# sikang/motion_primitive_library

Hardware: AMD Instinct MI355X
Metric: node-expansions/s (frontier x |U| pair evaluations per second) (higher is better)
Workload: dtype f64; 1 GPU; C4: 3D VoxelMapUtil 512^3, Control::ACC |U|=729 (9^3), 64k-node synthetic frontier; frontier=random, frontier_nodes=65536, frontier_nodes_per_gpu=65536, controls=729, dim=3, map_cells=134217728, device=AMD Radeon Graphics (gfx950:sramecc+:xnack-), compute_units=256, kernel=expand_lex_kernel

## Files before the change

motion_primitive_library_amd/build.py:

```python
import os
import shutil
import subprocess
import sys

HERE = os.path.dirname(os.path.abspath(__file__))
CSRC = os.path.join(HERE, "csrc")
LIB = os.path.join(CSRC, "libmplx.so")
SOURCES = ["expand_kernel.hip", "expand_tile_kernel.hip", "expand_grid_kernel.hip", "expand_lex_kernel.hip", "expand_pair_kernel.hip", "map_prep_kernel.hip", "map_prep_api.cpp", "map_util_kernel.hip", "map_util_api.cpp", "rollout_kernel.hip", "rollout_api.cpp", "ray_kernel.hip", "ray_api.cpp", "traj_kernel.hip", "traj_api.cpp", "solve_kernel.hip", "solve_api.cpp", "limits_kernel.hip", "limits_api.cpp", "scale_kernel.hip", "scale_api.cpp", "conflict_kernel.hip", "conflict_api.cpp", "reserve_kernel.hip", "reserve_api.cpp", "reserve_poly_kernel.hip", "reserve_poly_api.cpp", "wait_kernel.hip", "wait_api.cpp", "table_kernel.hip", "table_api.cpp", "open_kernel.hip", "open_best_kernel.hip", "open_rekey_kernel.hip", "open_api.cpp", "field_kernel.hip", "field_api.cpp", "heur_kernel.hip", "heur_api.cpp", "replan_kernel.hip", "replan_api.cpp", "post_kernel.hip", "identity_kernel.hip", "post_api.cpp", "edge_kernel.hip", "edge_api.cpp", "mplx_api.cpp", "lists_route.cpp", "yaw_pin.cpp", "lists_host.cpp", "planner_capi.cpp", "pack_kernel.hip", "store_model_kernel.hip", "lists_copy_api.cpp", "pack_api.cpp", "comm_api.cpp"]
HEADERS = ["mplx_internal.h", "mplx_ctx.h", "mplx_stage.h", "mplx_device_common.h", "mplx_pair_device.h", "mplx_grid_common.h", "mplx_poly.h", "mplx_traj_device.h", "mplx_limits_math.h", "mplx_scale_math.h", "mplx_heur_math.h", "mplx_open_heur.h", "host_planner.hpp", "host_lpastar.hpp", os.path.join("..", "..", "include", "mplx.h"), os.path.join("..", "..", "include", "mplx_debug.h"), os.path.join("..", "..", "include", "mplx_map_util.h"), os.path.join("..", "..", "include", "mplx_rollout.h"), os.path.join("..", "..", "include", "mplx_ray.h"), os.path.join("..", "..", "include", "mplx_traj.h"), os.path.join("..", "..", "include", "mplx_table.h"), os.path.join("..", "..", "include", "mplx_open.h"), os.path.join("..", "..", "include", "mplx_multi.h"), os.path.join("..", "..", "include", "mplx_replan.h"), os.path.join("..", "..", "include", "mplx_replan_timed.h"), os.path.join("..", "..", "include", "mplx_prior.h"), os.path.join("..", "..", "include", "mplx_solve.h"), os.path.join("..", "..", "include", "mplx_limits.h"), os.path.join("..", "..", "include", "mplx_scale.h"), os.path.join("..", "..", "include", "mplx_conflict.h"), os.path.join("..", "..", "include", "mplx_reserve.h"), os.path.join("..", "..", "include", "mplx_reserve_poly.h"), os.path.join("..", "..", "include", "mplx_wait.h"), os.path.join("..", "..", "include", "mplx_field.h"), os.path.join("..", "..", "include", "mplx_heur.h"), os.path.join("..", "..", "include", "mplx_best.h"), os.path.join("..", "..", "include", "mplx_anytime.h")]
ARCH = "gfx950"


def hipcc_path():
    for cand in (os.environ.get("HIPCC"), shutil.which("hipcc"), "/opt/rocm/bin/hipcc"):
        if cand and os.path.exists(cand):
            return cand
    raise RuntimeError("hipcc not found (set HIPCC or install ROCm under /opt/rocm)")


def _obj_dir():
    d = os.path.join(CSRC, "build")
    os.makedirs(d, exist_ok=True)
    return d


def is_stale():
    if not os.path.exists(LIB):
        return True
    t = os.path.getmtime(LIB)
    deps = [os.path.join(CSRC, s) for s in SOURCES + HEADERS]
    return any(os.path.getmtime(d) > t for d in deps)

# ... 61 lines not shown
```

motion_primitive_library_amd/csrc/expand_lex_kernel.hip:

```cpp
#include "mplx_internal.h"
#include "mplx_device_common.h"

namespace mplx {

using namespace dev;

constexpr int kLexWPB = 4;
constexpr int kLexBT = 64 * kLexWPB;
constexpr int kLexTabStride = 64;
constexpr int kLexUB8 = 8;

constexpr int kShUval = 0;
__host__ __device__ constexpr int lex_sh_tc(int TS) { return TS == 32 ? 768 : 384; }
__host__ __device__ constexpr int lex_sh_tt(int TS) { return lex_sh_tc(TS) + 64; }
__host__ __device__ constexpr int lex_ts(int ndp) { return ndp <= 8 ? 8 : (ndp <= 16 ? 16 : 32); }

__host__ __device__ constexpr int lex_fixed_bytes(int D, int K, int TS) {
  const int F = 4 * D + 2, KQ = K == 3 ? 4 : K;
  int w = (F * 8 + 15) & ~15;
  w += 128 + D * TS * 4 + D * TS * 4 * KQ + D * TS * 8 * (K - 1) + (K == 3 ? D * TS * 8 : 0) + D * TS + D * TS;
  w = (w + 15) & ~15;
  return (w + 128 + 7) & ~7;
}
__host__ __device__ constexpr int lex_tt_entries(int n_max) { return (n_max + 1) * (n_max + 2) / 2; }
// ... 511 lines not shown
        for (int i = 0; i < D; i++) {
          lo[i] = wave_reduce_minmax<false>(lo_l[i]);
          const int hi = wave_reduce_minmax<true>(hi_l[i]);
          if (hi < lo[i]) have_box = false;
          nb[i] = hi - lo[i] + 1;
        }
      }
      lex_sync();
      const int WX = (nb[0] + 31) >> 5;
      const int n_rows = nb[1] * nb[2];
      const bool fits = have_box && n_rows * WX <= A.boxcap;
      const int rot = (WX == 1) ? (lo[0] & 31) : 0;
      if (D == 2 && eager) {
        if (fits && pass == 0 && lane < nb[1]) {
          unsigned int val = e_in ? (__builtin_amdgcn_alignbit(e_a1, e_a0, e_shf) | ~e_mask) : 0xffffffffu;
          val = __builtin_amdgcn_alignbit(val, val, (32 - rot) & 31);
          s_box[lane] = val;
        }
      } else if (fits) {
        const float inv_ny = __builtin_amdgcn_rcpf((float)nb[1]);
        const int ax0 = base_c[0] + lo[0] - half;
        constexpr int SU = 4;
        const int ayb = base_c[1] + lo[1] - half, azb = (D == 3) ? base_c[2] + lo[2] - half : 0;
        for (int w = 0; w < WX; w++) {
          const int xw = ax0 + 32 * w;
          const int vlo = xw < 0 ? -xw : 0;
          const int vhi = (dims[0] - xw) < 32 ? (dims[0] - xw) : 32;
          const unsigned int mask = (vhi >= 32 ? 0xffffffffu : ((1u << (vhi > 0 ? vhi : 0)) - 1u)) & ~((1u << vlo) - 1u);
          for (int r0 = lane; r0 < n_rows; r0 += 64 * SU) {
            unsigned int a0[SU], a1[SU], shf[SU];
            bool in[SU];
#pragma unroll
            for (int u = 0; u < SU; u++) {
              const int r = r0 + 64 * u;
              const int rz = (D == 3) ? (int)(((float)r + 0.5f) * inv_ny) : 0;
              const int ry = r - rz * nb[1];
              const int ay = ayb + ry, az = azb + rz;
              in[u] = r < n_rows && vhi > vlo && ay >= 0 && ay < dims[1] && (D == 2 || (az >= 0 && az < dims[2]));
              const int64_t off = in[u] ? ((int64_t)az * dims[1] + ay) * (int64_t)dims[0] + xw : 0;
              const int64_t wi = off >> 5;
              shf[u] = (unsigned)(off & 31);
              const int64_t w0 = wi < 0 ? 0 : wi;
              const int64_t w1 = wi + 1 >= A.blk_words ? A.blk_words - 1 : wi + 1;
              a0[u] = (A.dbg & 8) ? 0u : A.blk[w0];
              a1[u] = (A.dbg & 8) ? 0u : A.blk[w1 < 0 ? 0 : w1];
            }
// ... 305 lines not shown
```

motion_primitive_library_amd/csrc/lists_route.cpp:

```cpp
#include "mplx_ctx.h"

#include <cmath>
#include <cstdio>
#include <cstdlib>

namespace mplx_detail {


template <class Args>
static void set_env(const mplx_ctx *c, Args *a) {
  a->region = c->has_region ? (const uint32_t *)c->region_bits.p : nullptr;
  a->dim0 = c->mdim[0]; a->dim1 = c->mdim[1]; a->dim2 = c->mdim[2];
  a->org0 = c->origin[0]; a->org1 = c->origin[1]; a->org2 = c->origin[2];
  a->res = c->res;
  a->dt = c->prm.dt; a->w = c->prm.w;
  a->v_max = c->prm.v_max; a->a_max = c->prm.a_max; a->j_max = c->prm.j_max;
}

template <class Args>
static void set_tables(const mplx_ctx *c, Args *a) {
  a->ttab = (const double *)c->tables.p;
  a->tcnt = (const unsigned char *)c->tables.p + kTcntOffset;
  a->Rres = c->recips[0]; a->R001 = c->recips[1]; a->R01 = c->recips[2];
}
// ... 306 lines not shown
  a->live_n = live_n;
  return MPLX_OK;
}

static int rebuild_sat(mplx_ctx *c) {
  c->sat_stale = false;
  const int d2p = c->dim == 3 ? c->mdim[2] + 1 : 2;
  const int64_t sat_n = (int64_t)(c->mdim[0] + 1) * (c->mdim[1] + 1) * d2p;
  if (c->tune.no_sat || sat_n * 4 > (16LL << 30)) return MPLX_OK;
  if (int rc = ensure(c, c->sat, (size_t)sat_n * 4)) return rc;
  HIP_TRY(c, mplx::launch_build_sat(c->dim, (const uint32_t *)c->blk.p, c->mdim, (uint32_t *)c->sat.p, c->stream));
  c->sat_ok = true;
  return MPLX_OK;
}

int ensure_blocked_bits(mplx_ctx *c) {
  if (c->blk_ok) return MPLX_OK;
  c->sat_stale = false;
  const int64_t words = (c->n_cells + 31) >> 5;
  if (int rc = ensure(c, c->blk, (size_t)words * 4)) return rc;
  HIP_TRY(c, mplx::launch_build_blocked_bits((const int8_t *)(c->has_pot ? c->pot.p : c->map.p),
                                             c->has_region ? (const uint32_t *)c->region_bits.p : nullptr, c->n_cells,
                                             c->has_pot ? 1 : 0, (uint32_t *)c->blk.p, c->stream));
  c->sat_ok = false;
  if (int rc = rebuild_sat(c)) return rc;
  c->blk_ok = true;
  return MPLX_OK;
}

int ensure_tables(mplx_ctx *c) {
  if (c->tables_ok && c->tab_dt == c->prm.dt && c->tab_res == c->res) return MPLX_OK;
  const size_t bytes = kTcntOffset + 64 + 64;
  if (int rc = ensure(c, c->tables, bytes)) return rc;
  double *ttab = (double *)c->tables.p;
  unsigned char *tcnt = (unsigned char *)c->tables.p + kTcntOffset;
  double *rec = (double *)((unsigned char *)c->tables.p + kTcntOffset + 64);
  HIP_TRY(c, hipMemsetAsync(c->tables.p, 0, bytes, c->stream));
  HIP_TRY(c, mplx::launch_make_tables(c->prm.dt, c->res, ttab, tcnt, rec, c->stream));
  HIP_TRY(c, hipMemcpyAsync(c->recips, rec, 3 * sizeof(double), hipMemcpyDeviceToHost, c->stream));
  HIP_TRY(c, hipStreamSynchronize(c->stream));
  c->tab_dt = c->prm.dt;
  c->tab_res = c->res;
  c->tables_ok = true;
  return MPLX_OK;
}

static uint32_t const_zero_rows(int dim, int control) {
  const int order = control_order(control);
  uint32_t m = 0;
  for (int b = order + 1; b <= 3; b++)
    for (int i = 0; i < dim; i++) m |= 1u << (b * dim + i);
  if (!(control & 0x10)) m |= 1u << (4 * dim);
  return m;
}

static mplx::GridArgs grid_args(mplx_ctx *c, const GridPlan &gp, const double *d_nodes, int64_t n_nodes, int64_t node_stride,
                                const mplx_succ_lists *o, uint32_t skip) {
  mplx::GridArgs a{};
  set_env(c, &a);
  set_tables(c, &a);
  set_lists(c, o, &a);
  a.blk = (const uint32_t *)c->blk.p;
  a.blk_words = (c->n_cells + 31) >> 5;
  a.pot = c->has_pot ? (const int8_t *)c->pot.p : nullptr;
  a.pot_w = c->prm.potential_weight;
  a.grad_w = c->has_pot ? c->prm.gradient_weight : 0.0;
  const bool yaw = (c->prm.control & 0x10) != 0;
  a.sat = (c->sat_ok && gp.order <= 3 && !(yaw && c->prm.wyaw > 0) && !c->tune.no_sat && gp.use_sat)
              ? (const uint32_t *)c->sat.p : nullptr;
  a.gather = gp.gather ? 1 : 0;
  a.yaw_max = c->prm.yaw_max; a.wyaw = c->prm.wyaw; a.ndy = yaw ? c->u_nd[3] : 0;
  a.uvals = (const double *)c->uvals.p + (c->u_wide ? 4 * 16 : 0);
  a.uval_stride = c->u_wide ? 32 : 16;
  a.uidx = (const uint32_t *)c->uidx.p;
  a.nd0 = c->u_nd[0]; a.nd1 = c->u_nd[1]; a.nd2 = c->u_nd[2];
  a.ndp = gp.ndp;
  a.ulex = gp.ulex;
  a.nU = c->nU;
  a.nodes = d_nodes; a.n_nodes = n_nodes; a.node_stride = node_stride;
  a.n_max = gp.n_max; a.rmax = gp.rmax; a.boxcap = gp.boxcap; a.grid_limit = gp.grid;
  a.lex = gp.lex ? 1 : 0;
  a.dbg = c->tune.dbg;
  a.l_pad = line_pad(c, a.l_nstride);
  a.l_zrows = skip;
  a.post = post_of(c, o);
  return a;
// ... 178 lines not shown
```

motion_primitive_library_amd/csrc/map_prep_api.cpp:

```cpp
#include "mplx_ctx.h"

#include <array>
#include <cmath>
#include <cstring>
#include <unordered_map>
#include <vector>

using namespace mplx_detail;

namespace {

inline int float_to_int(double pt, double origin, double res) { return (int)std::round((pt - origin) / res - 0.5); }

}

extern "C" {

int mplx_edit_map(mplx_ctx *c, const int64_t *cell_index, const int8_t *values, int64_t n) {
  if (!c) return MPLX_ERR_ARG;
  if (n < 0 || (n > 0 && (!cell_index || !values))) return fail(c, MPLX_ERR_ARG, "mplx_edit_map: bad arguments");
  if (!c->has_map) return fail(c, MPLX_ERR_STATE, "mplx_edit_map: set the map first");
  for (int64_t i = 0; i < n; i++)
    if (cell_index[i] < 0 || cell_index[i] >= c->n_cells)
      return fail(c, MPLX_ERR_ARG, "mplx_edit_map: cell index %lld outside the map of %lld cells", (long long)cell_index[i], (long long)c->n_cells);
// ... 8 lines not shown
        std::unordered_map<int64_t, int64_t> last;
        last.reserve((size_t)n * 2);
        for (int64_t i = 0; i < n; i++) last[cell_index[i]] = i;
        if ((int64_t)last.size() < n) {
          u_idx.reserve(last.size());
          u_val.reserve(last.size());
          for (int64_t i = 0; i < n; i++)
            if (last[cell_index[i]] == i) { u_idx.push_back(cell_index[i]); u_val.push_back(values[i]); }
          cell_index = u_idx.data();
          values = u_val.data();
          n = (int64_t)u_idx.size();
        }
      } catch (...) { return fail(c, MPLX_ERR_NOMEM, "mplx_edit_map: out of host memory"); }
    }
  }
  if (int rc = bind_device(c)) return rc;
  if (int rc = resolve_pending(c)) return rc;
  if (int rc = svc_stop(c)) return rc;
  StageRows s;
  const auto i_idx = s.in(cell_index, (size_t)n * 8), i_val = s.in(values, (size_t)n);
  if (int rc = stage_commit(c, &s)) return rc;
  c->map_upload_bytes += (uint64_t)n * 9;
  uint32_t *blk = (c->blk_ok && !c->has_pot) ? (uint32_t *)c->blk.p : nullptr;
  HIP_TRY(c, mplx::launch_edit_map(s.dev<int64_t>(i_idx), s.dev<int8_t>(i_val), n, c->n_cells, (int8_t *)c->map.p, blk,
                                   c->has_region ? (const uint32_t *)c->region_bits.p : nullptr, c->stream));
  if (int rc = stage_fetch(c, &s)) return rc;
  c->blk_epoch++;
  if (blk && c->sat_ok) {
    c->sat_ok = false;
    c->sat_stale = true;
  }
  return MPLX_OK;
}

int mplx_read_cells(mplx_ctx *c, int which, const int64_t *cell_index, int64_t n, int8_t *out) {
  if (!c) return MPLX_ERR_ARG;
  if (n < 0 || (n > 0 && (!cell_index || !out)) || (which != 0 && which != 1)) return fail(c, MPLX_ERR_ARG, "mplx_read_cells: bad arguments");
  if (which == 0 ? !c->has_map : !c->has_pot) return fail(c, MPLX_ERR_STATE, which == 0 ? "mplx_read_cells: no map set" : "mplx_read_cells: no potential map set");
  for (int64_t i = 0; i < n; i++)
    if (cell_index[i] < 0 || cell_index[i] >= c->n_cells)
      return fail(c, MPLX_ERR_ARG, "mplx_read_cells: cell index %lld outside the map of %lld cells", (long long)cell_index[i], (long long)c->n_cells);
  if (n == 0) return MPLX_OK;
  if (int rc = bind_device(c)) return rc;
  StageRows s;
  const auto i_idx = s.in(cell_index, (size_t)n * 8), o_val = s.out(out, (size_t)n);
  if (int rc = stage_commit(c, &s)) return rc;
  HIP_TRY(c, mplx::launch_gather_cells((const int8_t *)(which == 0 ? c->map.p : c->pot.p), s.dev<int64_t>(i_idx), n, s.dev<int8_t>(o_val), c->stream));
// ... 153 lines not shown
```

motion_primitive_library_amd/csrc/map_prep_kernel.hip:

```cpp
#include "mplx_internal.h"

namespace mplx {
namespace {

constexpr unsigned short kFar = 0xffff;

__global__ void pot_x_kernel(const int8_t *map, int d0, int d1, int d2, int c1x, int c2x, int c1y, int c2y, int c1z,
                             int c2z, int rn, unsigned short *dx2) {
  const int64_t n = (int64_t)d0 * d1 * d2;
  const int64_t g = (int64_t)blockIdx.x * blockDim.x + threadIdx.x;
  if (g >= n) return;
  const int x = (int)(g % d0);
  const int64_t row = g / d0;
  const int y = (int)(row % d1), z = (int)(row / d1);
  unsigned int best = kFar;
  if (y >= c1y && y < c2y && z >= c1z && z < c2z) {
    const int lo = max(x - rn, c1x), hi = min(x + rn, c2x - 1);
    const int8_t *r = map + row * d0;
    for (int s = lo; s <= hi; s++)
      if (r[s] > 0) {
        const unsigned int d = (unsigned)((s - x) * (s - x));
        best = d < best ? d : best;
      }
  }
// ... 52 lines not shown
  if (g >= per * n_cells_path) return;
  const int p = (int)(g / per);
  int64_t o = g - (int64_t)p * per;
  const int ox = (int)(o % bx) - rn0;
  o /= bx;
  const int oy = (int)(o % by) - rn1;
  const int oz = (int)(o / by) - rn2;
  const int x = cells[p * 3 + 0] + ox, y = cells[p * 3 + 1] + oy, z = (dim == 3) ? cells[p * 3 + 2] + oz : 0;
  if (x < 0 || x >= d0 || y < 0 || y >= d1 || z < 0 || z >= d2) return;
  const int64_t idx = x + (int64_t)d0 * y + (int64_t)d0 * d1 * z;
  atomicOr(&bits[idx >> 5], 1u << (idx & 31));
}

__global__ void unpack_region_kernel(const uint32_t *bits, int64_t n_cells, uint8_t *bytes) {
  const int64_t g = (int64_t)blockIdx.x * blockDim.x + threadIdx.x;
  if (g >= n_cells) return;
  bytes[g] = (uint8_t)((bits[g >> 5] >> (g & 31)) & 1u);
}

inline unsigned blocks_for(int64_t n) { return (unsigned)((n + 255) / 256); }


__global__ void edit_map_kernel(const int64_t *idx, const int8_t *val, int64_t n, int64_t n_cells, int8_t *map, uint32_t *blk,
                                const uint32_t *region) {
  const int64_t g = (int64_t)blockIdx.x * blockDim.x + threadIdx.x;
  if (g >= n) return;
  const int64_t c = idx[g];
  if (c < 0 || c >= n_cells) return;
  const int8_t v = val[g];
  map[c] = v;
  if (blk) {
    const uint32_t bit = 1u << (c & 31);
    const bool in_region = !region || ((region[c >> 5] >> (c & 31)) & 1u);
    if (v == 100 || !in_region) atomicOr(&blk[c >> 5], bit);
    else atomicAnd(&blk[c >> 5], ~bit);
  }
}

}

hipError_t launch_potential_passes(const int8_t *map, const int32_t *d, const int32_t *c1, const int32_t *c2, int rn,
                                   int hn, const int8_t *lut, int8_t h_max, unsigned short *tmp_a,
                                   unsigned short *tmp_b, int8_t *out, hipStream_t s) {
  const int64_t n = (int64_t)d[0] * d[1] * d[2];
  hipLaunchKernelGGL(pot_x_kernel, dim3(blocks_for(n)), dim3(256), 0, s, map, d[0], d[1], d[2], c1[0], c2[0], c1[1],
                     c2[1], c1[2], c2[2], rn, tmp_a);
  hipLaunchKernelGGL(pot_y_kernel, dim3(blocks_for(n)), dim3(256), 0, s, tmp_a, d[0], d[1], d[2], rn, tmp_b);
  hipLaunchKernelGGL(pot_z_kernel, dim3(blocks_for(n)), dim3(256), 0, s, map, tmp_b, lut, d[0], d[1], d[2], c1[0],
                     c2[0], c1[1], c2[1], c1[2], c2[2], hn, h_max, out);
  return hipGetLastError();
}

hipError_t launch_region_boxes(const int *cells, int n_path_cells, int dim, const int32_t *d, const int32_t *rn,
                               uint32_t *bits, hipStream_t s) {
  const int64_t per = (int64_t)(2 * rn[0] + 1) * (2 * rn[1] + 1) * (2 * rn[2] + 1);
  const int64_t total = per * n_path_cells;
  if (total == 0) return hipSuccess;
  hipLaunchKernelGGL(region_box_kernel, dim3(blocks_for(total)), dim3(256), 0, s, cells, n_path_cells, dim, d[0], d[1],
                     d[2], rn[0], rn[1], rn[2], bits);
  return hipGetLastError();
}

hipError_t launch_edit_map(const int64_t *idx, const int8_t *val, int64_t n, int64_t n_cells, int8_t *map, uint32_t *blk,
                           const uint32_t *region, hipStream_t s) {
  if (n == 0) return hipSuccess;
  hipLaunchKernelGGL(edit_map_kernel, dim3(blocks_for(n)), dim3(256), 0, s, idx, val, n, n_cells, map, blk, region);
  return hipGetLastError();
}

__global__ void gather_cells_kernel(const int8_t *cells, const int64_t *idx, int64_t n, int8_t *out) {
  const int64_t i = (int64_t)blockIdx.x * blockDim.x + threadIdx.x;
  if (i < n) out[i] = cells[idx[i]];
}

hipError_t launch_gather_cells(const int8_t *cells, const int64_t *idx, int64_t n, int8_t *out, hipStream_t s) {
  if (n == 0) return hipSuccess;
  hipLaunchKernelGGL(gather_cells_kernel, dim3(blocks_for(n)), dim3(256), 0, s, cells, idx, n, out);
  return hipGetLastError();
}

hipError_t launch_unpack_region(const uint32_t *bits, int64_t n_cells, uint8_t *bytes, hipStream_t s) {
  hipLaunchKernelGGL(unpack_region_kernel, dim3(blocks_for(n_cells)), dim3(256), 0, s, bits, n_cells, bytes);
  return hipGetLastError();
}

}
```

motion_primitive_library_amd/csrc/mplx_api.cpp:

```cpp
#include "mplx_ctx.h"
#include "host_planner.hpp"

#include <cmath>
#include <cstdio>
#include <cstdlib>
#include <cstring>
#include <new>
#include <string>
#include <vector>

using namespace mplx_detail;

namespace mplx_detail {
std::string &create_error() {
  thread_local std::string e;
  return e;
}

int ctx_ready(mplx_ctx *c) {
  if (!c->has_map) return fail(c, MPLX_ERR_STATE, "mplx_set_map has not been called");
  if (!c->has_params) return fail(c, MPLX_ERR_STATE, "mplx_set_params has not been called");
  if (!c->has_U) return fail(c, MPLX_ERR_STATE, "mplx_set_controls has not been called");
  const int need = c->dim + ((c->prm.control & 0x10) ? 1 : 0);
  if (c->udim < need)
// ... 70 lines not shown
      c->n_cus = prop.multiProcessorCount;
  }
  {
    auto env_int = [](const char *name) { const char *e = getenv(name); return e ? atoi(e) : 0; };
    c->tune.grid_rmax = env_int("MPLX_GRID_RMAX");
    c->tune.grid_boxcap = env_int("MPLX_GRID_BOXCAP");
    c->tune.grid_blocks = env_int("MPLX_GRID_BLOCKS");
    c->tune.grid_waves_per_cu = env_int("MPLX_GRID_WAVES_PER_CU");
    c->tune.grid_static = getenv("MPLX_GRID_STATIC") != nullptr;
    if (getenv("MPLX_GRID_LEX")) c->tune.grid_lex = env_int("MPLX_GRID_LEX") != 0;
    c->tune.grid_chunk = env_int("MPLX_GRID_CHUNK");
    c->tune.grid_blocked = env_int("MPLX_GRID_BLOCKED");
    c->tune.grid_gather = getenv("MPLX_GRID_GATHER") ? env_int("MPLX_GRID_GATHER") : -1;
    c->tune.grid_sat = getenv("MPLX_GRID_SAT") ? env_int("MPLX_GRID_SAT") : -1;
    c->tune.dbg = env_int("MPLX_TILE_DBG");
    c->tune.no_pair = getenv("MPLX_GRID_PAIR") && env_int("MPLX_GRID_PAIR") == 0;
    c->tune.pair_rmax = env_int("MPLX_PAIR_RMAX");
    c->tune.pair_wg_per_cu = env_int("MPLX_PAIR_WG_PER_CU");
    c->tune.arena_kb = env_int("MPLX_ARENA_KB");
    c->tune.zero_copy = getenv("MPLX_ZERO_COPY") ? env_int("MPLX_ZERO_COPY") : 1;
    c->tune.no_sat = getenv("MPLX_GRID_NOSAT") != nullptr;
    c->tune.no_lex = getenv("MPLX_GRID_NOLEX") != nullptr;
    c->tune.no_line_pad = getenv("MPLX_NO_LINE_PAD") != nullptr;
    c->tune.prescreen_min = env_int("MPLX_GRID_PRESCREEN_MIN");
    c->tune.yaw_pin = !(getenv("MPLX_YAW_PIN") && atoi(getenv("MPLX_YAW_PIN")) == 0);
    c->tune.yaw_margin = getenv("MPLX_YAW_MARGIN") ? atof(getenv("MPLX_YAW_MARGIN")) : 0.0;
    if (getenv("MPLX_SERVICE")) c->tune.service = env_int("MPLX_SERVICE");
    if (getenv("MPLX_DONE_FLAG")) c->tune.done_flag = env_int("MPLX_DONE_FLAG");
    if (env_int("MPLX_SERVICE_IDLE_US") > 0) c->tune.service_idle_us = env_int("MPLX_SERVICE_IDLE_US");
    if (env_int("MPLX_SERVICE_MAX_NODES") > 0) c->tune.service_max_nodes = env_int("MPLX_SERVICE_MAX_NODES");
    if (env_int("MPLX_RESERVE_LANES") > 0) c->tune.reserve_lanes = env_int("MPLX_RESERVE_LANES");
  }
  if (c->tune.done_flag) {
    e = hipHostMalloc((void **)&c->done_host, 64, hipHostMallocCoherent);
    if (e == hipSuccess) { *c->done_host = 0; e = hipMalloc(&c->done_count.p, 64); }
    if (e == hipSuccess) { c->done_count.cap = 64; e = hipMemset(c->done_count.p, 0, 64); }
    if (e != hipSuccess) {
      fail(nullptr, MPLX_ERR_HIP, "mplx_create: HIP set-up of the completion word failed: %s", hipGetErrorString(e));
      mplx_destroy(c);
      return MPLX_ERR_HIP;
    }
  }
  if (c->tune.service) {
    mplx_ctx::Service &sv = c->svc;
    e = hipStreamCreateWithFlags(&sv.stream, hipStreamNonBlocking);
    if (e == hipSuccess) e = hipHostMalloc((void **)&sv.mb, sizeof(mplx::SvcMailbox), hipHostMallocCoherent);
// ... 8 lines not shown
    if (e == hipSuccess) sv.dev.cap = 1025 * 8;
    if (e != hipSuccess) {
      fail(nullptr, MPLX_ERR_HIP, "mplx_create: HIP set-up of the service failed: %s", hipGetErrorString(e));
      mplx_destroy(c);
      return MPLX_ERR_HIP;
    }
  }
  *out = c;
  return MPLX_OK;
}

void mplx_destroy(mplx_ctx *c) {
  if (!c) return;
  (void)hipSetDevice(c->device);
  (void)mplx_detail::svc_stop(c);
  if (c->svc.stream) (void)hipStreamDestroy(c->svc.stream);
  if (c->svc.mb) (void)hipHostFree(c->svc.mb);
  if (c->svc.block) (void)hipHostFree(c->svc.block);
  release(c->svc.dev);
  if (c->stream) (void)hipStreamSynchronize(c->stream);
  if (c->done_host) (void)hipHostFree(c->done_host);
  release(c->done_count);
  for (DevBuf *b : {&c->map, &c->pot, &c->region_bits, &c->region_bytes, &c->U, &c->tables,
                    &c->d_status, &c->d_cost, &c->d_hash, &c->d_state, &c->d_iters, &c->uvals, &c->uidx, &c->blk, &c->sat, &c->prep_lut, &c->prep_a, &c->prep_b, &c->post_keys, &c->post_ws, &c->ray_work, &c->heur_ws, &c->traj_tab, &c->conflict_ws, &c->live_list, &c->live_ctr})
    release(*b);
  (void)mplx_comm_destroy(c);
  release(c->comm_meta);
  c->yaw_pending.clear();
  for (DevBuf *b : {&c->yaw_ring, &c->yaw_ids, &c->yaw_tab, &c->work_counter}) release(*b);
  if (c->yaw_any_host) (void)hipHostFree(c->yaw_any_host);
  if (c->id_ovf_host) (void)hipHostFree(c->id_ovf_host);
  mplx_detail::release_copy_buffers(c);
  release(c->s_arena);
  if (c->h_arena) (void)hipHostFree(c->h_arena);
  if (c->ev0) (void)hipEventDestroy(c->ev0);
  if (c->ev1) (void)hipEventDestroy(c->ev1);
  if (c->stream) (void)hipStreamDestroy(c->stream);
  delete c;
}

int mplx_set_map(mplx_ctx *c, const int8_t *cells, const int32_t *dim, const double *origin, double res) {
  if (!c) return MPLX_ERR_ARG;
  if (!cells || !dim || !origin) return fail(c, MPLX_ERR_ARG, "mplx_set_map: NULL argument");
  if (!(res > 0)) return fail(c, MPLX_ERR_ARG, "mplx_set_map: resolution must be > 0");
  int64_t n = 1;
  for (int i = 0; i < c->dim; i++) {
    if (dim[i] <= 0) return fail(c, MPLX_ERR_ARG, "mplx_set_map: dim[%d] = %d", i, dim[i]);
// ... 386 lines not shown
```

motion_primitive_library_amd/csrc/mplx_ctx.h:

```cpp
#ifndef MPLX_CTX_H
#define MPLX_CTX_H

#include "../../include/mplx.h"
#include "../../include/mplx_debug.h"
#include "../../include/mplx_open.h"
#include "../../include/mplx_traj.h"
#include "mplx_internal.h"
#include "mplx_stage.h"

#include <cstdarg>
#include <cstdio>
#include <exception>
#include <new>
#include <string>
#include <vector>

struct mplx_table;
struct mplx_reserve;

namespace mplx_detail {

struct DevBuf {
  void *p = nullptr;
  size_t cap = 0;
// ... 4 lines not shown
}

struct mplx_ctx {
  int dim = 0;
  int device = 0;
  hipStream_t stream = nullptr;
  hipEvent_t ev0 = nullptr, ev1 = nullptr;
  std::string err;

  mplx_detail::DevBuf map, pot, region_bits, region_bytes, U;
  bool has_map = false, has_pot = false, has_region = false, has_params = false, has_U = false;
  bool has_goal = false;
  mplx::PostFuse goal_fuse{};
  int32_t goal_ctl[2] = {0, 0};
  int32_t mdim[3] = {1, 1, 1};
  double origin[3] = {0, 0, 0};
  double res = 0;
  int64_t n_cells = 0;
  uint64_t map_upload_bytes = 0;
  mplx_params prm{};
  int32_t nU = 0, udim = 0;
  double u_absmax = 0;
  mplx_detail::DevBuf uvals, uidx, blk, sat;
  bool sat_ok = false;
  mplx_detail::DevBuf post_keys;
  mplx_detail::DevBuf post_ws;
  mplx_detail::DevBuf ray_work;
  mplx_detail::DevBuf heur_ws;
  mplx_detail::DevBuf traj_tab;
  mplx_detail::DevBuf conflict_ws;
  mplx_detail::DevBuf prep_lut, prep_a, prep_b;
  bool blk_ok = false;
  uint64_t blk_epoch = 0;
  bool u_factored = false;
  bool u_wide = false;
  bool u_lex = false;
  int32_t u_nd[4] = {0, 0, 0, 0};
  struct Tuning {
    int grid_rmax = 0, grid_boxcap = 0, grid_blocks = 0;
    int grid_waves_per_cu = 0;
    int grid_gather = -1, grid_sat = -1;
    bool grid_lex = true;
    bool grid_static = false;
    int grid_chunk = 0;
    int grid_blocked = 0;
    int dbg = 0;
    bool no_pair = false;
    int pair_rmax = 0, pair_wg_per_cu = 0;
    int zero_copy = 1;
    int arena_kb = 0;
    bool no_sat = false, no_lex = false, no_line_pad = false;
    int prescreen_min = 0;
    bool yaw_pin = true;
    double yaw_margin = 0;
    int done_flag = 1;
    int service = 1;
    int service_idle_us = 500;
    int service_max_nodes = 256;
    int reserve_lanes = 0;
  } tune;
  int lists_route = MPLX_ROUTE_AUTO;
  int last_route = MPLX_ROUTE_AUTO;
  uint32_t last_zero_rows = 0;
  bool last_grid_pair = false;
  bool last_grid_lex = false;
  int n_cus = 256;

  mplx_detail::DevBuf tables;
  bool tables_ok = false;
  double tab_dt = 0, tab_res = 0;
  double recips[3] = {0, 0, 0};
  mplx_detail::DevBuf d_status, d_cost, d_hash, d_state, d_iters;
  mplx_detail::DevBuf s_arena;
  void *h_arena = nullptr;
// ... 240 lines not shown
```

motion_primitive_library_amd/csrc/mplx_internal.h:

```cpp
#ifndef MPLX_INTERNAL_H
#define MPLX_INTERNAL_H

#include <hip/hip_runtime.h>
#include <stdint.h>

namespace mplx {

struct YawPin {
  int32_t *amb;
  int32_t *any_host;
  int32_t amb_cap;
  double margin;
  double tie_yaw;
  const int32_t *node_list;
  const double *tab;
  int32_t tab_stride;
  double cos_lim;
};

struct ExpandArgs {
  const int8_t *map;
  const int8_t *pot;
  const uint32_t *region;
  int32_t dim0, dim1, dim2;
// ... 71 lines not shown
  double *l_state;
  int64_t l_stride;
  int32_t *l_iters;
  int64_t l_nstride;
  int32_t l_pad;
  PostFuse post;
  SvcMailbox *svc_mb;
  uint64_t *svc_dev;
  uint64_t svc_seq0;
  uint64_t svc_idle;
  DoneSignal done;
};

size_t tile_lds_bytes(int tile_pairs, int npb, int wl_cap, int n_max, int n_fields, int u_doubles,
                      int *u_offset);
hipError_t launch_make_tables(double T, double res, double *ttab, unsigned char *tcnt, double *recips,
                              hipStream_t stream);
hipError_t launch_expand_tile(int dim, int control, const TileArgs &args, hipStream_t stream);
int tile_service_resident_workgroups(int dim, int control, const TileArgs &a);

struct GridArgs {
  const uint32_t *blk;
  int64_t blk_words;
  const int8_t *pot;
  const uint32_t *region;
  double pot_w, grad_w;
  const uint32_t *sat;
  int32_t dim0, dim1, dim2;
  double org0, org1, org2;
  double res;
  double dt, w;
  double v_max, a_max, j_max;
  double yaw_max, wyaw;
  const double *uvals;
  int32_t uval_stride;
  const uint32_t *uidx;
  int32_t nd0, nd1, nd2;
  int32_t ndy;
  int32_t ulex;
  int32_t ndp;
  int32_t nU;
  const double *nodes;
  int64_t n_nodes, node_stride;
  int32_t n_max;
  int32_t rmax;
  int32_t boxcap;
// ... 41 lines not shown
  int64_t dst_off[kPackRows];
  int32_t es[kPackRows];
  int32_t n_rows;
  int64_t node_stride;
  const int32_t *count;
  const int64_t *offs;
  int64_t node0, off0;
  char *dst;
};
hipError_t launch_pack_rows(const PackArgs &args, int64_t n_nodes, hipStream_t stream);
hipError_t launch_scan_counts(const int32_t *count, int64_t n, int64_t *offs, hipStream_t stream);
size_t grid_lds_bytes(int dim, int order, int nU, int ndp, int n_max, int rmax, int boxcap, int yaw_mode, int ndy,
                      int ulex);
int grid_waves_per_block();
int grid_resident_blocks(int dim, int control, bool pot, size_t lds);
hipError_t launch_expand_grid(int dim, int control, const GridArgs &args, hipStream_t stream);
bool lex_covers(int dim, int control);
size_t lex_lds_bytes(int dim, int order, int ndp, int nU, int n_max, int rmax, int boxcap);
int lex_waves_per_block();
int lex_resident_blocks(int dim, int control, int ndp, size_t lds);
hipError_t launch_expand_lex(int dim, int control, const GridArgs &args, hipStream_t stream);
hipError_t launch_gather_cells(const int8_t *cells, const int64_t *idx, int64_t n, int8_t *out, hipStream_t s);
hipError_t launch_edit_map(const int64_t *idx, const int8_t *val, int64_t n, int64_t n_cells, int8_t *map, uint32_t *blk,
                           const uint32_t *region, hipStream_t s);
int64_t dilate_words_per_row(int32_t d0);
hipError_t launch_dilate(int8_t *map, const int32_t *d, const void *runs, int n_runs, uint32_t *bits, hipStream_t s);
hipError_t launch_free_unknown(int8_t *map, int64_t n_cells, hipStream_t s);
hipError_t launch_cloud_count(const int8_t *map, int dim, const int32_t *d, int kind, int32_t *count, int64_t *offs,
                              hipStream_t s);
hipError_t launch_cloud_fill(const int8_t *map, int dim, const int32_t *d, int kind, const int64_t *offs, int64_t lo,
                             int64_t hi, double res, const double *origin, double *xyz, hipStream_t s);
hipError_t launch_build_sat(int dim, const uint32_t *blk, const int32_t *mdim, uint32_t *sat, hipStream_t stream);
hipError_t launch_build_blocked_bits(const int8_t *map, const uint32_t *region, int64_t n_cells, int potential,
                                     uint32_t *out, hipStream_t stream);

hipError_t launch_store_model(const int32_t *count, int64_t n_nodes, int64_t S, int32_t *action, double *cost, uint64_t *hash,
                              double *state, int64_t state_stride, int n_fields, int pad, int blocks, int mode,
                              uint32_t skip_rows, hipStream_t s);

struct EdgeArgs {
  const int8_t *map;
  const uint32_t *region;
  int32_t dim0, dim1, dim2;
  double org0, org1, org2;
  double res;
  double dt, w;
  const double *U;
// ... 664 lines not shown
```

Baseline: 109.3 billion pairs/s.

## Add 3D brick layout for blocked-bit map and gather lex boxes from bricks

Adds a secondary copy of the 3D blocked-bit map stored in 32x4x4 bricks: 16 dwords each, with 4 y-rows per 16-byte quad. The copy is built once after map prep and kept in sync on map edits. The lex expansion kernel then fills its LDS occupancy box by loading uint4 quads covering four y rows per lane, replacing per-row dword gathers. This is meant to cut scattered global loads and improve locality when building the collision box. In exchange it costs extra device memory, a build pass, and extra atomics on edits.

```diff
diff --git a/motion_primitive_library_amd/build.py b/motion_primitive_library_amd/build.py
--- a/motion_primitive_library_amd/build.py
+++ b/motion_primitive_library_amd/build.py
@@ -7,7 +7,7 @@
 CSRC = os.path.join(HERE, "csrc")
 LIB = os.path.join(CSRC, "libmplx.so")
 SOURCES = ["expand_kernel.hip", "expand_tile_kernel.hip", "expand_grid_kernel.hip", "expand_lex_kernel.hip", "expand_pair_kernel.hip", "map_prep_kernel.hip", "map_prep_api.cpp", "map_util_kernel.hip", "map_util_api.cpp", "rollout_kernel.hip", "rollout_api.cpp", "ray_kernel.hip", "ray_api.cpp", "traj_kernel.hip", "traj_api.cpp", "solve_kernel.hip", "solve_api.cpp", "limits_kernel.hip", "limits_api.cpp", "scale_kernel.hip", "scale_api.cpp", "conflict_kernel.hip", "conflict_api.cpp", "reserve_kernel.hip", "reserve_api.cpp", "reserve_poly_kernel.hip", "reserve_poly_api.cpp", "wait_kernel.hip", "wait_api.cpp", "table_kernel.hip", "table_api.cpp", "open_kernel.hip", "open_best_kernel.hip", "open_rekey_kernel.hip", "open_api.cpp", "field_kernel.hip", "field_api.cpp", "heur_kernel.hip", "heur_api.cpp", "replan_kernel.hip", "replan_api.cpp", "post_kernel.hip", "identity_kernel.hip", "post_api.cpp", "edge_kernel.hip", "edge_api.cpp", "mplx_api.cpp", "lists_route.cpp", "yaw_pin.cpp", "lists_host.cpp", "planner_capi.cpp", "pack_kernel.hip", "store_model_kernel.hip", "lists_copy_api.cpp", "pack_api.cpp", "comm_api.cpp"]
-HEADERS = ["mplx_internal.h", "mplx_ctx.h", "mplx_stage.h", "mplx_device_common.h", "mplx_pair_device.h", "mplx_grid_common.h", "mplx_poly.h", "mplx_traj_device.h", "mplx_limits_math.h", "mplx_scale_math.h", "mplx_heur_math.h", "mplx_open_heur.h", "host_planner.hpp", "host_lpastar.hpp", os.path.join("..", "..", "include", "mplx.h"), os.path.join("..", "..", "include", "mplx_debug.h"), os.path.join("..", "..", "include", "mplx_map_util.h"), os.path.join("..", "..", "include", "mplx_rollout.h"), os.path.join("..", "..", "include", "mplx_ray.h"), os.path.join("..", "..", "include", "mplx_traj.h"), os.path.join("..", "..", "include", "mplx_table.h"), os.path.join("..", "..", "include", "mplx_open.h"), os.path.join("..", "..", "include", "mplx_multi.h"), os.path.join("..", "..", "include", "mplx_replan.h"), os.path.join("..", "..", "include", "mplx_replan_timed.h"), os.path.join("..", "..", "include", "mplx_prior.h"), os.path.join("..", "..", "include", "mplx_solve.h"), os.path.join("..", "..", "include", "mplx_limits.h"), os.path.join("..", "..", "include", "mplx_scale.h"), os.path.join("..", "..", "include", "mplx_conflict.h"), os.path.join("..", "..", "include", "mplx_reserve.h"), os.path.join("..", "..", "include", "mplx_reserve_poly.h"), os.path.join("..", "..", "include", "mplx_wait.h"), os.path.join("..", "..", "include", "mplx_field.h"), os.path.join("..", "..", "include", "mplx_heur.h"), os.path.join("..", "..", "include", "mplx_best.h"), os.path.join("..", "..", "include", "mplx_anytime.h")]
+HEADERS = ["mplx_internal.h", "mplx_ctx.h", "mplx_stage.h", "mplx_device_common.h", "mplx_pair_device.h", "mplx_grid_common.h", "mplx_brick.h", "mplx_poly.h", "mplx_traj_device.h", "mplx_limits_math.h", "mplx_scale_math.h", "mplx_heur_math.h", "mplx_open_heur.h", "host_planner.hpp", "host_lpastar.hpp", os.path.join("..", "..", "include", "mplx.h"), os.path.join("..", "..", "include", "mplx_debug.h"), os.path.join("..", "..", "include", "mplx_map_util.h"), os.path.join("..", "..", "include", "mplx_rollout.h"), os.path.join("..", "..", "include", "mplx_ray.h"), os.path.join("..", "..", "include", "mplx_traj.h"), os.path.join("..", "..", "include", "mplx_table.h"), os.path.join("..", "..", "include", "mplx_open.h"), os.path.join("..", "..", "include", "mplx_multi.h"), os.path.join("..", "..", "include", "mplx_replan.h"), os.path.join("..", "..", "include", "mplx_replan_timed.h"), os.path.join("..", "..", "include", "mplx_prior.h"), os.path.join("..", "..", "include", "mplx_solve.h"), os.path.join("..", "..", "include", "mplx_limits.h"), os.path.join("..", "..", "include", "mplx_scale.h"), os.path.join("..", "..", "include", "mplx_conflict.h"), os.path.join("..", "..", "include", "mplx_reserve.h"), os.path.join("..", "..", "include", "mplx_reserve_poly.h"), os.path.join("..", "..", "include", "mplx_wait.h"), os.path.join("..", "..", "include", "mplx_field.h"), os.path.join("..", "..", "include", "mplx_heur.h"), os.path.join("..", "..", "include", "mplx_best.h"), os.path.join("..", "..", "include", "mplx_anytime.h")]
 ARCH = "gfx950"
 
 
diff --git a/motion_primitive_library_amd/csrc/expand_lex_kernel.hip b/motion_primitive_library_amd/csrc/expand_lex_kernel.hip
--- a/motion_primitive_library_amd/csrc/expand_lex_kernel.hip
+++ b/motion_primitive_library_amd/csrc/expand_lex_kernel.hip
@@ -1,5 +1,6 @@
 #include "mplx_internal.h"
 #include "mplx_device_common.h"
+#include "mplx_brick.h"
 
 namespace mplx {
 
@@ -557,6 +558,61 @@
         const int ax0 = base_c[0] + lo[0] - half;
         constexpr int SU = 4;
         const int ayb = base_c[1] + lo[1] - half, azb = (D == 3) ? base_c[2] + lo[2] - half : 0;
+        if (D == 3 && A.blk_brick != nullptr) {
+          const int bbx = A.bbx, bby = A.bby;
+          const int qy0 = ayb >> 2;
+          const int nq = ((ayb + nb[1] - 1) >> 2) - qy0 + 1;
+          const int n_items = nq * nb[2];
+          const float inv_nq = __builtin_amdgcn_rcpf((float)nq);
+          const unsigned int xsh = (unsigned)ax0 & 31u;
+          const uint4 ones4 = make_uint4(0xffffffffu, 0xffffffffu, 0xffffffffu, 0xffffffffu);
+          constexpr int SQ = K == 3 ? 1 : 2;
+          for (int w = 0; w < WX; w++) {
+            const int xw = ax0 + 32 * w;
+            const int vlo = xw < 0 ? -xw : 0;
+            const int vhi = (dims[0] - xw) < 32 ? (dims[0] - xw) : 32;
+            const unsigned int mask = (vhi >= 32 ? 0xffffffffu : ((1u << (vhi > 0 ? vhi : 0)) - 1u)) & ~((1u << vlo) - 1u);
+            const int X0 = xw >> 5;
+            const int span = (nb[0] - 32 * w) < 32 ? (nb[0] - 32 * w) : 32;
+            const bool two = (int)xsh + span > 32;
+            const bool x0_in = X0 >= 0 && X0 < bbx, x1_in = X0 + 1 >= 0 && X0 + 1 < bbx;
+            for (int i0 = lane; i0 < n_items; i0 += 64 * SQ) {
+              uint4 q0[SQ], q1[SQ];
+              int rz_[SQ], yq_[SQ];
+#pragma unroll
+              for (int u = 0; u < SQ; u++) {
+                const int i = i0 + 64 * u;
+                const int rz = (int)(((float)i + 0.5f) * inv_nq);
+                const int yq = qy0 + (i - rz * nq), az = azb + rz;
+                const bool in = i < n_items && yq >= 0 && yq < bby && az >= 0 && az < dims[2];
+                rz_[u] = rz;
+                yq_[u] = yq;
+                const bool in0 = in && x0_in;
+                const uint4 v = *(const uint4 *)(A.blk_brick + (in0 ? brick_quad(bbx, bby, X0, yq, az) : 0));
+                q0[u] = in0 ? ((A.dbg & 8) ? make_uint4(0u, 0u, 0u, 0u) : v) : ones4;
+                q1[u] = ones4;
+                if (two) {
+                  const bool in1 = in && x1_in;
+                  const uint4 v1 = *(const uint4 *)(A.blk_brick + (in1 ? brick_quad(bbx, bby, X0 + 1, yq, az) : 0));
+                  q1[u] = in1 ? ((A.dbg & 8) ? make_uint4(0u, 0u, 0u, 0u) : v1) : ones4;
+                }
+              }
+#pragma unroll
+              for (int u = 0; u < SQ; u++) {
+                const int i = i0 + 64 * u;
+                const unsigned int a0[4] = {q0[u].x, q0[u].y, q0[u].z, q0[u].w}, a1[4] = {q1[u].x, q1[u].y, q1[u].z, q1[u].w};
+                const int ry0 = 4 * yq_[u] - ayb;
+#pragma unroll
+                for (int j = 0; j < 4; j++) {
+                  unsigned int val = __builtin_amdgcn_alignbit(a1[j], a0[j], xsh) | ~mask;
+                  val = __builtin_amdgcn_alignbit(val, val, (32 - rot) & 31);
+                  const int ry = ry0 + j;
+                  if (i < n_items && ry >= 0 && ry < nb[1]) s_box[(rz_[u] * nb[1] + ry) * WX + w] = val;
+                }
+              }
+            }
+          }
+        } else
         for (int w = 0; w < WX; w++) {
           const int xw = ax0 + 32 * w;
           const int vlo = xw < 0 ? -xw : 0;
diff --git a/motion_primitive_library_amd/csrc/lists_route.cpp b/motion_primitive_library_amd/csrc/lists_route.cpp
--- a/motion_primitive_library_amd/csrc/lists_route.cpp
+++ b/motion_primitive_library_amd/csrc/lists_route.cpp
@@ -1,4 +1,5 @@
 #include "mplx_ctx.h"
+#include "mplx_brick.h"
 
 #include <cmath>
 #include <cstdio>
@@ -352,6 +353,11 @@
   HIP_TRY(c, mplx::launch_build_blocked_bits((const int8_t *)(c->has_pot ? c->pot.p : c->map.p),
                                              c->has_region ? (const uint32_t *)c->region_bits.p : nullptr, c->n_cells,
                                              c->has_pot ? 1 : 0, (uint32_t *)c->blk.p, c->stream));
+  if (c->dim == 3 && !c->has_pot) {
+    const mplx::BrickGrid bg = mplx::brick_grid(c->mdim[0], c->mdim[1], c->mdim[2]);
+    if (int rc = ensure(c, c->blk_brick, (size_t)mplx::brick_dwords(bg) * 4)) return rc;
+    HIP_TRY(c, mplx::launch_build_bricks((const uint32_t *)c->blk.p, words, c->mdim, (uint32_t *)c->blk_brick.p, c->stream));
+  }
   c->sat_ok = false;
   if (int rc = rebuild_sat(c)) return rc;
   c->blk_ok = true;
@@ -392,6 +398,11 @@
   set_lists(c, o, &a);
   a.blk = (const uint32_t *)c->blk.p;
   a.blk_words = (c->n_cells + 31) >> 5;
+  if (c->dim == 3 && !c->has_pot && c->tune.grid_brick && c->blk_brick.p) {
+    const mplx::BrickGrid bg = mplx::brick_grid(c->mdim[0], c->mdim[1], c->mdim[2]);
+    a.blk_brick = (const uint32_t *)c->blk_brick.p;
+    a.bbx = bg.bx; a.bby = bg.by; a.bbz = bg.bz;
+  }
   a.pot = c->has_pot ? (const int8_t *)c->pot.p : nullptr;
   a.pot_w = c->prm.potential_weight;
   a.grad_w = c->has_pot ? c->prm.gradient_weight : 0.0;
diff --git a/motion_primitive_library_amd/csrc/map_prep_api.cpp b/motion_primitive_library_amd/csrc/map_prep_api.cpp
--- a/motion_primitive_library_amd/csrc/map_prep_api.cpp
+++ b/motion_primitive_library_amd/csrc/map_prep_api.cpp
@@ -54,7 +54,8 @@
   if (int rc = stage_commit(c, &s)) return rc;
   c->map_upload_bytes += (uint64_t)n * 9;
   uint32_t *blk = (c->blk_ok && !c->has_pot) ? (uint32_t *)c->blk.p : nullptr;
-  HIP_TRY(c, mplx::launch_edit_map(s.dev<int64_t>(i_idx), s.dev<int8_t>(i_val), n, c->n_cells, (int8_t *)c->map.p, blk,
+  uint32_t *brick = (blk && c->dim == 3) ? (uint32_t *)c->blk_brick.p : nullptr;
+  HIP_TRY(c, mplx::launch_edit_map(s.dev<int64_t>(i_idx), s.dev<int8_t>(i_val), n, c->n_cells, (int8_t *)c->map.p, blk, brick, c->mdim,
                                    c->has_region ? (const uint32_t *)c->region_bits.p : nullptr, c->stream));
   if (int rc = stage_fetch(c, &s)) return rc;
   c->blk_epoch++;
diff --git a/motion_primitive_library_amd/csrc/map_prep_kernel.hip b/motion_primitive_library_amd/csrc/map_prep_kernel.hip
--- a/motion_primitive_library_amd/csrc/map_prep_kernel.hip
+++ b/motion_primitive_library_amd/csrc/map_prep_kernel.hip
@@ -1,4 +1,5 @@
 #include "mplx_internal.h"
+#include "mplx_brick.h"
 
 namespace mplx {
 namespace {
@@ -98,7 +99,7 @@
 
 
 __global__ void edit_map_kernel(const int64_t *idx, const int8_t *val, int64_t n, int64_t n_cells, int8_t *map, uint32_t *blk,
-                                const uint32_t *region) {
+                                uint32_t *brick, int d0, int d1, int d2, const uint32_t *region) {
   const int64_t g = (int64_t)blockIdx.x * blockDim.x + threadIdx.x;
   if (g >= n) return;
   const int64_t c = idx[g];
@@ -108,9 +109,27 @@
   if (blk) {
     const uint32_t bit = 1u << (c & 31);
     const bool in_region = !region || ((region[c >> 5] >> (c & 31)) & 1u);
-    if (v == 100 || !in_region) atomicOr(&blk[c >> 5], bit);
+    const bool blocked = v == 100 || !in_region;
+    if (blocked) atomicOr(&blk[c >> 5], bit);
     else atomicAnd(&blk[c >> 5], ~bit);
+    if (brick) {
+      const int64_t row = c / d0;
+      const int x = (int)(c - row * d0), y = (int)(row % d1), z = (int)(row / d1);
+      const BrickGrid bg = brick_grid(d0, d1, d2);
+      uint32_t *w = &brick[brick_dword(bg.bx, bg.by, x >> 5, y, z)];
+      if (blocked) atomicOr(w, 1u << (x & 31));
+      else atomicAnd(w, ~(1u << (x & 31)));
+    }
   }
+}
+
+__global__ void build_bricks_kernel(const uint32_t *blk, int64_t blk_words, int d0, int d1, int d2, int bx, int by,
+                                    int64_t n_dwords, uint32_t *brick) {
+  const int64_t g = (int64_t)blockIdx.x * blockDim.x + threadIdx.x;
+  if (g >= n_dwords) return;
+  int xw, y, z;
+  brick_row_of(bx, by, g, &xw, &y, &z);
+  brick[g] = brick_word_from_rows(blk, blk_words, d0, d1, d2, xw, y, z);
 }
 
 }
@@ -138,9 +157,18 @@
 }
 
 hipError_t launch_edit_map(const int64_t *idx, const int8_t *val, int64_t n, int64_t n_cells, int8_t *map, uint32_t *blk,
-                           const uint32_t *region, hipStream_t s) {
+                           uint32_t *brick, const int32_t *d, const uint32_t *region, hipStream_t s) {
   if (n == 0) return hipSuccess;
-  hipLaunchKernelGGL(edit_map_kernel, dim3(blocks_for(n)), dim3(256), 0, s, idx, val, n, n_cells, map, blk, region);
+  hipLaunchKernelGGL(edit_map_kernel, dim3(blocks_for(n)), dim3(256), 0, s, idx, val, n, n_cells, map, blk, blk ? brick : nullptr,
+                     d[0], d[1], d[2], region);
+  return hipGetLastError();
+}
+
+hipError_t launch_build_bricks(const uint32_t *blk, int64_t blk_words, const int32_t *d, uint32_t *brick, hipStream_t s) {
+  const BrickGrid bg = brick_grid(d[0], d[1], d[2]);
+  const int64_t n = brick_dwords(bg);
+  hipLaunchKernelGGL(build_bricks_kernel, dim3(blocks_for(n)), dim3(256), 0, s, blk, blk_words, d[0], d[1], d[2], bg.bx, bg.by, n,
+                     brick);
   return hipGetLastError();
 }
 
diff --git a/motion_primitive_library_amd/csrc/mplx_api.cpp b/motion_primitive_library_amd/csrc/mplx_api.cpp
--- a/motion_primitive_library_amd/csrc/mplx_api.cpp
+++ b/motion_primitive_library_amd/csrc/mplx_api.cpp
@@ -116,6 +116,7 @@
     c->tune.no_sat = getenv("MPLX_GRID_NOSAT") != nullptr;
     c->tune.no_lex = getenv("MPLX_GRID_NOLEX") != nullptr;
     c->tune.no_line_pad = getenv("MPLX_NO_LINE_PAD") != nullptr;
+    if (getenv("MPLX_GRID_BRICK")) c->tune.grid_brick = env_int("MPLX_GRID_BRICK") != 0;
     c->tune.prescreen_min = env_int("MPLX_GRID_PRESCREEN_MIN");
     c->tune.yaw_pin = !(getenv("MPLX_YAW_PIN") && atoi(getenv("MPLX_YAW_PIN")) == 0);
     c->tune.yaw_margin = getenv("MPLX_YAW_MARGIN") ? atof(getenv("MPLX_YAW_MARGIN")) : 0.0;
@@ -170,7 +171,7 @@
   if (c->done_host) (void)hipHostFree(c->done_host);
   release(c->done_count);
   for (DevBuf *b : {&c->map, &c->pot, &c->region_bits, &c->region_bytes, &c->U, &c->tables,
-                    &c->d_status, &c->d_cost, &c->d_hash, &c->d_state, &c->d_iters, &c->uvals, &c->uidx, &c->blk, &c->sat, &c->prep_lut, &c->prep_a, &c->prep_b, &c->post_keys, &c->post_ws, &c->ray_work, &c->heur_ws, &c->traj_tab, &c->conflict_ws, &c->live_list, &c->live_ctr})
+                    &c->d_status, &c->d_cost, &c->d_hash, &c->d_state, &c->d_iters, &c->uvals, &c->uidx, &c->blk, &c->blk_brick, &c->sat, &c->prep_lut, &c->prep_a, &c->prep_b, &c->post_keys, &c->post_ws, &c->ray_work, &c->heur_ws, &c->traj_tab, &c->conflict_ws, &c->live_list, &c->live_ctr})
     release(*b);
   (void)mplx_comm_destroy(c);
   release(c->comm_meta);
diff --git a/motion_primitive_library_amd/csrc/mplx_brick.h b/motion_primitive_library_amd/csrc/mplx_brick.h
--- /dev/null
+++ b/motion_primitive_library_amd/csrc/mplx_brick.h
@@ -0,0 +1,55 @@
+#ifndef MPLX_BRICK_H
+#define MPLX_BRICK_H
+
+#include <cstdint>
+
+#if defined(__HIPCC__) || defined(__CUDACC__)
+#define MPLX_BRICK_HD __host__ __device__
+#else
+#define MPLX_BRICK_HD
+#endif
+
+namespace mplx {
+
+constexpr int kBrickDwords = 16;
+
+struct BrickGrid {
+  int32_t bx, by, bz;
+};
+MPLX_BRICK_HD inline BrickGrid brick_grid(int32_t d0, int32_t d1, int32_t d2) {
+  return BrickGrid{(d0 + 31) >> 5, (d1 + 3) >> 2, (d2 + 3) >> 2};
+}
+MPLX_BRICK_HD inline int64_t brick_dwords(const BrickGrid &g) { return (int64_t)g.bx * g.by * g.bz * kBrickDwords; }
+
+MPLX_BRICK_HD inline int64_t brick_dword(int32_t bx, int32_t by, int32_t xw, int32_t y, int32_t z) {
+  return (((int64_t)(z >> 2) * by + (y >> 2)) * bx + xw) * kBrickDwords + (z & 3) * 4 + (y & 3);
+}
+MPLX_BRICK_HD inline int64_t brick_quad(int32_t bx, int32_t by, int32_t xw, int32_t yq, int32_t z) {
+  return (((int64_t)(z >> 2) * by + yq) * bx + xw) * kBrickDwords + (z & 3) * 4;
+}
+
+MPLX_BRICK_HD inline void brick_row_of(int32_t bx, int32_t by, int64_t g, int32_t *xw, int32_t *y, int32_t *z) {
+  const int32_t in = (int32_t)(g & (kBrickDwords - 1));
+  int64_t b = g >> 4;
+  *xw = (int32_t)(b % bx);
+  b /= bx;
+  *y = (int32_t)(b % by) * 4 + (in & 3);
+  *z = (int32_t)(b / by) * 4 + (in >> 2);
+}
+
+MPLX_BRICK_HD inline uint32_t brick_word_from_rows(const uint32_t *blk, int64_t words, int32_t d0, int32_t d1, int32_t d2,
+                                                  int32_t xw, int32_t y, int32_t z) {
+  if (y >= d1 || z >= d2) return 0xffffffffu;
+  const int64_t off = ((int64_t)z * d1 + y) * (int64_t)d0 + 32 * (int64_t)xw;
+  const int64_t wi = off >> 5;
+  const int sh = (int)(off & 31);
+  const uint32_t a0 = blk[wi];
+  const uint32_t a1 = (sh && wi + 1 < words) ? blk[wi + 1] : 0u;
+  uint32_t v = sh ? ((a0 >> sh) | (a1 << (32 - sh))) : a0;
+  const int left = d0 - 32 * xw;
+  if (left < 32) v |= ~((1u << left) - 1u);
+  return v;
+}
+
+}
+#endif
diff --git a/motion_primitive_library_amd/csrc/mplx_ctx.h b/motion_primitive_library_amd/csrc/mplx_ctx.h
--- a/motion_primitive_library_amd/csrc/mplx_ctx.h
+++ b/motion_primitive_library_amd/csrc/mplx_ctx.h
@@ -50,6 +50,7 @@
   int32_t nU = 0, udim = 0;
   double u_absmax = 0;
   mplx_detail::DevBuf uvals, uidx, blk, sat;
+  mplx_detail::DevBuf blk_brick;
   bool sat_ok = false;
   mplx_detail::DevBuf post_keys;
   mplx_detail::DevBuf post_ws;
@@ -78,6 +79,7 @@
     int zero_copy = 1;
     int arena_kb = 0;
     bool no_sat = false, no_lex = false, no_line_pad = false;
+    bool grid_brick = true;
     int prescreen_min = 0;
     bool yaw_pin = true;
     double yaw_margin = 0;
diff --git a/motion_primitive_library_amd/csrc/mplx_internal.h b/motion_primitive_library_amd/csrc/mplx_internal.h
--- a/motion_primitive_library_amd/csrc/mplx_internal.h
+++ b/motion_primitive_library_amd/csrc/mplx_internal.h
@@ -117,6 +117,8 @@
 struct GridArgs {
   const uint32_t *blk;
   int64_t blk_words;
+  const uint32_t *blk_brick;
+  int32_t bbx, bby, bbz;
   const int8_t *pot;
   const uint32_t *region;
   double pot_w, grad_w;
@@ -204,7 +206,8 @@
 hipError_t launch_expand_lex(int dim, int control, const GridArgs &args, hipStream_t stream);
 hipError_t launch_gather_cells(const int8_t *cells, const int64_t *idx, int64_t n, int8_t *out, hipStream_t s);
 hipError_t launch_edit_map(const int64_t *idx, const int8_t *val, int64_t n, int64_t n_cells, int8_t *map, uint32_t *blk,
-                           const uint32_t *region, hipStream_t s);
+                           uint32_t *brick, const int32_t *d, const uint32_t *region, hipStream_t s);
+hipError_t launch_build_bricks(const uint32_t *blk, int64_t blk_words, const int32_t *d, uint32_t *brick, hipStream_t s);
 int64_t dilate_words_per_row(int32_t d0);
 hipError_t launch_dilate(int8_t *map, const int32_t *d, const void *runs, int n_runs, uint32_t *bits, hipStream_t s);
 hipError_t launch_free_unknown(int8_t *map, int64_t n_cells, hipStream_t s);
diff --git a/profiles/micro/brick_ab.py b/profiles/micro/brick_ab.py
--- /dev/null
+++ b/profiles/micro/brick_ab.py
@@ -0,0 +1,55 @@
+import json
+import os
+import sys
+
+ROOT = os.path.dirname(os.path.dirname(os.path.dirname(os.path.abspath(__file__))))
+sys.path.insert(0, ROOT)
+import bench
+import motion_primitive_library_amd as m
+
+name = sys.argv[1] if len(sys.argv) > 1 else "C4"
+rounds = int(sys.argv[2]) if len(sys.argv) > 2 else 7
+K = int(sys.argv[3]) if len(sys.argv) > 3 else 20
+n_alloc = int(sys.argv[4]) if len(sys.argv) > 4 else 1
+wl = m.workloads.make(name, potential_fn=m.workloads.device_potential_fn(0) if name == "C5" else None)
+envs = {}
+for leg, flag in (("brick", "1"), ("rows", "0")):
+    os.environ["MPLX_GRID_BRICK"] = flag
+    envs[leg] = m.EnvMap(wl.dim, 0)
+    wl.apply(envs[leg])
+os.environ.pop("MPLX_GRID_BRICK")
+fr = envs["brick"].upload_frontier(wl.nodes)
+
+
+def timed(env, lists):
+    for _ in range(3):
+        env.expand_lists_resident(fr, lists)
+    env.synchronize()
+    env.timer_begin()
+    for _ in range(K):
+        env.expand_lists_resident(fr, lists)
+    return env.timer_end() / K
+
+
+def med(v):
+    v = sorted(v)
+    return v[len(v) // 2]
+
+
+for a in range(n_alloc):
+    lists = envs["brick"].alloc_lists(wl.n_nodes, want_state=True, want_iters=False)
+    spun = bench.spin_up(envs["rows"], fr, lists)
+    res = {"brick": [], "rows": []}
+    for r in range(rounds):
+        for leg in (("brick", "rows") if r % 2 == 0 else ("rows", "brick")):
+            res[leg].append(timed(envs[leg], lists))
+        if n_alloc == 1:
+            print(json.dumps({"round": r, "brick_ms": round(res["brick"][-1], 5), "rows_ms": round(res["rows"][-1], 5)}), flush=True)
+    print(json.dumps({
+        "workload": name, "kernel": envs["brick"].last_grid_kernel(), "allocation": a, "spin_up_launches": spun, "launches_per_leg": K,
+        "rounds": rounds,
+        "brick_ms": {"median": round(med(res["brick"]), 5), "min": round(min(res["brick"]), 5), "max": round(max(res["brick"]), 5)},
+        "rows_ms": {"median": round(med(res["rows"]), 5), "min": round(min(res["rows"]), 5), "max": round(max(res["rows"]), 5)},
+        "ratio_median": round(med(res["brick"]) / med(res["rows"]), 4), "ratio_min": round(min(res["brick"]) / min(res["rows"]), 4)}),
+        flush=True)
+    lists.free()
```

Result: no change. 109.8 billion pairs/s (median of 6 runs) (+0.5%).
